# nmwsharp/diffusion-net

Hardware: NVIDIA H100
Metric: DiffusionNetBlock forward Mverts/sec at V=200k,K=128,C=128; 1/2/4/8 GPU (higher is better)
Workload: dtype f32

## Files before the change

### diffusion-net_b200/csrc/dn_tc.cu

```cuda
#include "dn_internal.h"
#include "dn_tc_ptx.cuh"
#include <cuda.h>
#include <cudaTypedefs.h>
#include <cuda_bf16.h>
#include <string.h>

namespace {

using namespace tc;

constexpr int KC = 16;
constexpr int TILE_M = 128;
constexpr int W_RING_BYTES = 128 * 1024;
constexpr int W_NST_MAX = 8;
constexpr int CHAIN_THREADS = 384;
constexpr int A_BOX_BYTES = 8 * TILE_M * 4;
constexpr int A_STAGE_BYTES = 2 * A_BOX_BYTES;
constexpr int A_NST_MAX = 8;
constexpr int SMEM_OPTIN = 232448;
constexpr int OUT_ROWS = 64;
constexpr int OUT_BOX_BYTES = 8 * OUT_ROWS * 4;

enum { MODE_TF32 = 1, MODE_TF32X3 = 3, MODE_BF16 = DN_PASSES_BF16 };

// ... 420 lines not shown
            if (Lr.residual) {
              if (ok0) {
                const float2 r = __ldg(reinterpret_cast<const float2*>(Lr.residual + r0 * Lr.ld_res + col));
                v0.x = fmaf(Lr.res_scale, r.x, v0.x); v0.y = fmaf(Lr.res_scale, r.y, v0.y);
              }
              if (ok1) {
                const float2 r = __ldg(reinterpret_cast<const float2*>(Lr.residual + r1 * Lr.ld_res + col));
                v1.x = fmaf(Lr.res_scale, r.x, v1.x); v1.y = fmaf(Lr.res_scale, r.y, v1.y);
              }
            }
            if (Lr.out) {
              if (ok0) *reinterpret_cast<float2*>(Lr.out + r0 * Lr.ld_out + col) = v0;
              if (ok1) *reinterpret_cast<float2*>(Lr.out + r1 * Lr.ld_out + col) = v1;
            }
          }
          if constexpr (kChain) {
            if (!keep_act) {
              act[8 * j + 4 * h] = v0.x; act[8 * j + 4 * h + 1] = v0.y;
              act[8 * j + 4 * h + 2] = v1.x; act[8 * j + 4 * h + 3] = v1.y;
            }
          }
          if (!kChain && head) {
#pragma unroll
            for (int o = 0; o < (kChain ? 1 : 8); ++o) {
              if (o >= p.head_n) break;
              const float2 w = __ldg(reinterpret_cast<const float2*>(p.head_w + (int64_t)o * N + col));
              hp0[o] = fmaf(w.y, v0.y, fmaf(w.x, v0.x, hp0[o]));
              hp1[o] = fmaf(w.y, v1.y, fmaf(w.x, v1.x, hp1[o]));
            }
          }
        }
      }
      if constexpr (kStage) {
        if (Lr.out || Lr.residual) {
          fence_proxy_async();
          named_bar_sync(2 + wg, 128);
          if (Lr.out && elected && row0 < p.V) {
            for (int b = 0; b < Lr.N / 8; ++b)
              tma_tile_2d_s2g(&p.omap[l], 8 * b, row0, smem_u32(stg_box(b)));
            bulk_commit();
            if (tile + gridDim.x >= ntiles) bulk_wait<0>();
          }
        }
      }
      if (head) {
        auto head_store = [&](int o, float a0, float a1) {
          a0 += __shfl_xor_sync(0xffffffffu, a0, 1);
          a0 += __shfl_xor_sync(0xffffffffu, a0, 2);
          a1 += __shfl_xor_sync(0xffffffffu, a1, 1);
          a1 += __shfl_xor_sync(0xffffffffu, a1, 2);
          const float b = p.head_b ? __ldg(p.head_b + o) : 0.f;
          if (t == 0 && ok0) p.head_out[r0 * p.ld_head_out + o] = a0 + b;
          if (t == 0 && ok1) p.head_out[r1 * p.ld_head_out + o] = a1 + b;
        };
        if constexpr (kChain) {
#pragma unroll 1
          for (int o = 0; o < p.head_n; ++o) {
            float a0 = 0.f, a1 = 0.f;
#pragma unroll
            for (int j = 0; j < NB; ++j) {
              if (j >= nb) break;
#pragma unroll
              for (int h = 0; h < 2; ++h) {
                const float* v = act + 8 * j + 4 * h;
                const float2 w = __ldg(reinterpret_cast<const float2*>(p.head_w + (int64_t)o * N + 16 * j + 8 * h + 2 * t));
                a0 = fmaf(w.y, v[1], fmaf(w.x, v[0], a0));
                a1 = fmaf(w.y, v[3], fmaf(w.x, v[2], a1));
              }
            }
            head_store(o, a0, a1);
          }
        } else {
#pragma unroll
          for (int o = 0; o < (kChain ? 1 : 8); ++o) {
            if (o >= p.head_n) break;
            head_store(o, hp0[o], hp1[o]);
          }
        }
      }
    }
  }
}

constexpr int TB_NST = 4;
constexpr int TB_RAW_HALF = KC * 128 * 4;
constexpr int TB_RAW = 2 * TB_RAW_HALF;
constexpr int TB_BIMG = KC * 128 * 4;
constexpr int TB_BSTAGE = 2 * TB_BIMG;
constexpr int TB_THREADS = 288;
constexpr int TB_SUMS = 64 * 256 * 4;
constexpr int TB_SMEM = TB_NST * TB_RAW + 2 * TB_BSTAGE + TB_SUMS + 256;
constexpr int TB_FOLD = 8;

struct TcToBasisParams {
  const float* values;
  const float* basis;
  const float* mass;
  float* partial;
  int64_t V;
  int K, C;
  int64_t chunks_per_cta;
  int64_t ld_values;
  int64_t ldp;
  const int32_t* cta_rows;
};

template <int MODE, int NBC>
__global__ void __launch_bounds__(TB_THREADS, 1) to_basis_kernel(const __grid_constant__ TcToBasisParams p) {
  extern __shared__ __align__(1024) uint8_t smem[];
  uint8_t* raw = smem;
  uint8_t* bimg = smem + TB_NST * TB_RAW;
  float* sums = reinterpret_cast<float*>(bimg + 2 * TB_BSTAGE);
  uint64_t* bars = reinterpret_cast<uint64_t*>(bimg + 2 * TB_BSTAGE + TB_SUMS);
  const uint32_t st_full = smem_u32(bars), st_empty = smem_u32(bars + TB_NST);
  const int warp = threadIdx.x >> 5, lane = threadIdx.x & 31;
  if (threadIdx.x == 0) {
    for (int i = 0; i < TB_NST; ++i) { mbar_init(st_full + 8 * i, 1); mbar_init(st_empty + 8 * i, 8); }
    fence_barrier_init();
  }
  __syncthreads();

  int64_t rb, re;
  if (p.cta_rows) {
    rb = p.cta_rows[2 * blockIdx.x];
    re = p.cta_rows[2 * blockIdx.x + 1];
  } else {
    rb = (int64_t)blockIdx.x * p.chunks_per_cta * KC;
    re = rb + p.chunks_per_cta * KC;
    if (re > p.V) re = p.V;
  }
  const int64_t nch = re > rb ? (re - rb + KC - 1) / KC : 0;
  constexpr int C = 16 * NBC;
  const int K = p.K;

  if (warp == 8) {
    if (lane == 0) {
      for (int64_t c = 0; c < nch; ++c) {
        const uint32_t s = c % TB_NST, ph = (c / TB_NST) & 1;
        mbar_wait(st_empty + 8 * s, ph ^ 1);
        const int64_t v0 = rb + c * KC;
        const int nv = (int)((re - v0) < KC ? (re - v0) : KC);
        const uint32_t ba = (uint32_t)nv * K * 4, bb = (uint32_t)nv * C * 4;
        mbar_arrive_expect_tx(st_full + 8 * s, ba + bb);
        tma_bulk_g2s(smem_u32(raw + s * TB_RAW), p.basis + v0 * K, ba, st_full + 8 * s);
        if (p.ld_values == C) {
          tma_bulk_g2s(smem_u32(raw + s * TB_RAW + TB_RAW_HALF), p.values + v0 * C, bb, st_full + 8 * s);
        } else {
          for (int j = 0; j < nv; ++j)
            tma_bulk_g2s(smem_u32(raw + s * TB_RAW + TB_RAW_HALF) + (uint32_t)j * C * 4, p.values + (v0 + j) * p.ld_values,
                         (uint32_t)C * 4, st_full + 8 * s);
        }
      }
    }
    return;
  }

  const int g = lane >> 2, t = lane & 3;
  const int m0 = (warp >> 2) * 64 + (warp & 3) * 16 + g;
  const uint32_t lbo = (uint32_t)C * 16;
  float acc[64];
  float* sum = sums + threadIdx.x;
#pragma unroll
  for (int i = 0; i < 64; ++i) sum[256 * i] = 0.f;

  for (int64_t c = 0; c < nch; ++c) {
    const uint32_t s = c % TB_NST, ph = (c / TB_NST) & 1;
    const int64_t v0 = rb + c * KC;
    const int nv = (int)((re - v0) < KC ? (re - v0) : KC);
    const int fold = (int)(c % TB_FOLD);
    if (fold == 0 && c > 0) {
      wgmma_wait<0>();
#pragma unroll
      for (int j = 0; j < 8; ++j) fence_acc8(acc + 8 * j);
#pragma unroll
      for (int i = 0; i < 64; ++i) sum[256 * i] += acc[i];
    }
    float mv[NBC], xv[NBC];
    if (p.mass) {
#pragma unroll
      for (int i = 0; i < NBC; ++i) {
        const int vv = (256 * i + (int)threadIdx.x) / C;
        mv[i] = __ldg(p.mass + v0 + (vv < nv ? vv : nv - 1));
      }
    }
    named_bar_sync(1, 256);
    mbar_wait(st_full + 8 * s, ph);
    const float* rphi = reinterpret_cast<const float*>(raw + s * TB_RAW);
    const float* rx = reinterpret_cast<const float*>(raw + s * TB_RAW + TB_RAW_HALF);
    uint8_t* bh = bimg + (c & 1) * TB_BSTAGE;
#pragma unroll
    for (int i = 0; i < NBC; ++i) xv[i] = rx[256 * i + (int)threadIdx.x];
#pragma unroll
    for (int i = 0; i < NBC; ++i) {
      const int e = 256 * i + (int)threadIdx.x;
      const int vv = e / C, cc = e - vv * C;
      float x = 0.f;
      if (vv < nv) x = p.mass ? xv[i] * mv[i] : xv[i];
      float hi, lo;
      split_tf32_fast(x, hi, lo);
      const uint32_t off = (vv >> 2) * C * 16 + (cc >> 3) * 128 + (cc & 7) * 16 + (vv & 3) * 4;
      *reinterpret_cast<float*>(bh + off) = hi;
      if (MODE == MODE_TF32X3) *reinterpret_cast<float*>(bh + TB_BIMG + off) = lo;
    }
    wgmma_wait<0>();
    uint32_t ah[2][4], al[2][4];
#pragma unroll
    for (int ks = 0; ks < 2; ++ks)
#pragma unroll
      for (int i = 0; i < 4; ++i) {
        const int vv = 8 * ks + t + 4 * (i >> 1), k = m0 + 8 * (i & 1);
        const float v = rphi[vv * K + k];
        float h, lo;
        split_tf32_fast((vv < nv && k < K) ? v : 0.f, h, lo);
        ah[ks][i] = __float_as_uint(h);
        al[ks][i] = __float_as_uint(lo);
      }
    fence_proxy_async();
    __syncwarp();
    if (lane == 0) mbar_arrive(st_empty + 8 * s);
    named_bar_sync(2, 256);
    const uint32_t sb = smem_u32(bh);
#pragma unroll
    for (int ks = 0; ks < 2; ++ks) {
      fence_frag4(ah[ks]);
      if (MODE == MODE_TF32X3) fence_frag4(al[ks]);
    }
    wgmma_fence();
#pragma unroll
    for (int ks = 0; ks < 2; ++ks) {
      const uint32_t acc0 = (fold > 0 || ks > 0) ? 1u : 0u;
      if constexpr (NBC == 8) {
        const uint32_t base = sb + ks * 2 * lbo;
        const uint64_t dh = make_desc(base, lbo, 128);
        if (MODE == MODE_TF32X3) {
          wgmma_tf32_n128(acc, al[ks], dh, acc0);
          wgmma_tf32_n128(acc, ah[ks], make_desc(base + TB_BIMG, lbo, 128), 1u);
          wgmma_tf32_n128(acc, ah[ks], dh, 1u);
        } else {
          wgmma_tf32_n128(acc, ah[ks], dh, acc0);
        }
      } else {
#pragma unroll
        for (int j = 0; j < NBC; ++j) {
          const uint32_t base = sb + ks * 2 * lbo + j * 256;
          const uint64_t dh = make_desc(base, lbo, 128);
          if (MODE == MODE_TF32X3) {
            wgmma_tf32_n16(acc + 8 * j, al[ks], dh, acc0);
            wgmma_tf32_n16(acc + 8 * j, ah[ks], make_desc(base + TB_BIMG, lbo, 128), 1u);
            wgmma_tf32_n16(acc + 8 * j, ah[ks], dh, 1u);
          } else {
            wgmma_tf32_n16(acc + 8 * j, ah[ks], dh, acc0);
          }
        }
      }
    }
    wgmma_commit();
  }
  wgmma_wait<0>();
#pragma unroll
  for (int j = 0; j < 8; ++j) fence_acc8(acc + 8 * j);
  if (nch > 0)
#pragma unroll
    for (int i = 0; i < 64; ++i) sum[256 * i] += acc[i];
  float* out = p.partial + (int64_t)blockIdx.x * K * p.ldp;
#pragma unroll
  for (int b = 0; b < 16; ++b) {
    const int col = 8 * b + 2 * t;
    if (col >= C) break;
    if (m0 < K) *reinterpret_cast<float2*>(out + (int64_t)m0 * p.ldp + col) = make_float2(sum[256 * (4 * b)], sum[256 * (4 * b + 1)]);
    if (m0 + 8 < K)
      *reinterpret_cast<float2*>(out + (int64_t)(m0 + 8) * p.ldp + col) = make_float2(sum[256 * (4 * b + 2)], sum[256 * (4 * b + 3)]);
  }
}

constexpr int kMaxDev = 64;
struct DevState { int queried, sms, sm90, tc_tried, tc; };
DevState g_dev[kMaxDev];

template <typename F>
bool set_smem(F* f, int bytes) {
  return cudaFuncSetAttribute(f, cudaFuncAttributeMaxDynamicSharedMemorySize, bytes) == cudaSuccess;
}
template <int MODE, int NBC0 = 1>
bool set_to_basis_smem() {
  if constexpr (NBC0 > 8) return true;
  else return set_smem(to_basis_kernel<MODE, NBC0>, TB_SMEM) && set_to_basis_smem<MODE, NBC0 + 1>();
}
template <int MODE, int NBC0 = 1>
void launch_to_basis(int nbc, int grid, const TcToBasisParams& p, cudaStream_t st) {
  if constexpr (NBC0 <= 8) {
    if (nbc == NBC0) to_basis_kernel<MODE, NBC0><<<grid, TB_THREADS, TB_SMEM, st>>>(p);
    else launch_to_basis<MODE, NBC0 + 1>(nbc, grid, p, st);
  }
}
template <int MODE>
bool set_chain_smem() {
  constexpr int s128 = ChainRing<MODE, 128>::SMEM, s256 = ChainRing<MODE, 256>::SMEM;
  return set_smem(rows_chain_kernel<MODE, 128, false>, s128) && set_smem(rows_chain_kernel<MODE, 128, true>, s128) &&
         set_smem(rows_chain_kernel<MODE, 256, false>, s256) && set_smem(rows_chain_kernel<MODE, 256, true>, s256);
}

PFN_cuTensorMapEncodeTiled_v12000 tensor_map_encoder() {
  static const PFN_cuTensorMapEncodeTiled_v12000 fn = [] {
    void* f = nullptr;
    cudaDriverEntryPointQueryResult q;
    if (cudaGetDriverEntryPointByVersion("cuTensorMapEncodeTiled", &f, 12000, cudaEnableDefault, &q) != cudaSuccess ||
        q != cudaDriverEntryPointSuccess) {
      cudaGetLastError();
      f = nullptr;
    }
    return reinterpret_cast<PFN_cuTensorMapEncodeTiled_v12000>(f);
  }();
  return fn;
}

}

static DevState* cur_dev_state() {
  int dev = 0;
  if (cudaGetDevice(&dev) != cudaSuccess || dev < 0 || dev >= kMaxDev) {
    cudaGetLastError();
    return nullptr;
  }
  DevState& d = g_dev[dev];
  if (!d.queried) {
    d.queried = 1;
    int major = 0, minor = 0;
    if (cudaDeviceGetAttribute(&d.sms, cudaDevAttrMultiProcessorCount, dev) != cudaSuccess ||
        cudaDeviceGetAttribute(&major, cudaDevAttrComputeCapabilityMajor, dev) != cudaSuccess ||
        cudaDeviceGetAttribute(&minor, cudaDevAttrComputeCapabilityMinor, dev) != cudaSuccess) {
      cudaGetLastError();
      major = 0;
    }
    if (d.sms < 1) d.sms = 1;
    d.sm90 = major == 9 && minor == 0;
  }
  return &d;
}

int dn_sm_count() {
  const DevState* d = cur_dev_state();
  return d ? d->sms : 1;
}

// ... 99 lines not shown
  }
}

int tc_rows_chain(const DnRowsSrc& src, const DnLayer* layers_in, int n_layers, int64_t V, int passes, void* ws,
                  int64_t ws_bytes, cudaStream_t st) {
  if (V <= 0) return DN_OK;
  if (n_layers < 1 || n_layers > DN_MAX_LAYERS) return DN_ERR_INVALID_ARGUMENT;
  DnLayer layers[DN_MAX_LAYERS];
  bool packed = true;
  for (int l = 0; l < n_layers; ++l) {
    layers[l] = layers_in[l];
    packed = packed && layers[l].prepacked != nullptr;
  }
  if (!packed) {
    int rc = tc_pack_layers(layers, n_layers, ws, ws_bytes, nullptr, st);
    if (rc) return rc;
  }
  const bool bf16 = passes == DN_PASSES_BF16 && layers[0].pack_fmt == 2;
  if (passes == DN_PASSES_BF16 && !bf16) passes = 1;
  if (V >= (1ll << 31) - 256) return DN_ERR_UNSUPPORTED;
  HcParams p;
  memset(&p, 0, sizeof(p));
  p.src = src;
  p.n_layers = n_layers;
  p.V = V;
  p.tile_group = layers[0].tile_group;
  p.group_stride = layers[0].group_stride;
  const PFN_cuTensorMapEncodeTiled_v12000 encode = tensor_map_encoder();
  if (!encode) return DN_ERR_UNSUPPORTED;
  auto encode_rows = [&](CUtensorMap* m, const float* base, int width, int64_t ld, int box_rows) {
    const cuuint64_t dims[2] = {(cuuint64_t)width, (cuuint64_t)V};
    const cuuint64_t strides[1] = {(cuuint64_t)ld * 4};
    const cuuint32_t box[2] = {8, (cuuint32_t)box_rows}, estr[2] = {1, 1};
    return encode(m, CU_TENSOR_MAP_DATA_TYPE_FLOAT32, 2, const_cast<float*>(base), dims, strides, box, estr,
                  CU_TENSOR_MAP_INTERLEAVE_NONE, CU_TENSOR_MAP_SWIZZLE_NONE, CU_TENSOR_MAP_L2_PROMOTION_L2_256B,
                  CU_TENSOR_MAP_FLOAT_OOB_FILL_NONE) == CUDA_SUCCESS;
  };
  for (int s = 0; s < src.nsrc; ++s)
    if (!encode_rows(&p.amap[s], src.ptr[s], src.width[s], src.ld[s], TILE_M)) return DN_ERR_UNSUPPORTED;
  int nmax = 0, nmin = 1 << 30;
  for (int l = 0; l < n_layers; ++l) {
    const DnLayer& L = layers[l];
    HcLayer& T = p.layer[l];
    T.wpack = L.prepacked; T.bias = L.bias; T.emul = L.emul; T.relu_mask = L.relu_mask_src; T.row_scale = L.row_scale;
    T.residual = L.residual; T.ld_res = L.ld_res; T.res_scale = L.res_scale; T.out = L.out; T.ld_out = L.ld_out;
    T.K = L.K; T.N = L.N; T.relu = L.relu; T.sibling = L.sibling;
    if (L.N > nmax) nmax = L.N;
    if (L.N < nmin) nmin = L.N;
  }
  if (nmax <= 128 && !bf16)
    for (int l = 0; l < n_layers; ++l) {
      const DnLayer& L = layers[l];
      if (L.out && !encode_rows(&p.omap[l], L.out, L.N, L.ld_out, OUT_ROWS)) return DN_ERR_UNSUPPORTED;
      if (L.residual && !encode_rows(&p.rmap[l], L.residual, L.N, L.ld_res, OUT_ROWS)) return DN_ERR_UNSUPPORTED;
    }
  const bool wide = nmin == nmax && (nmax == 128 || nmax == 256);
  const DnLayer& Ll = layers[n_layers - 1];
  p.head_w = Ll.head_w; p.head_b = Ll.head_b; p.head_out = Ll.head_out; p.ld_head_out = Ll.ld_head_out; p.head_n = Ll.head_n;
  const int64_t ntiles = (V + TILE_M - 1) / TILE_M;
  const int sms = dn_sm_count();
  const int grid = (int)(ntiles < sms ? ntiles : sms);
  if (bf16) launch_chain<MODE_BF16>(p, nmax, wide, grid, st);
  else if (passes == 3) launch_chain<MODE_TF32X3>(p, nmax, wide, grid, st);
  else launch_chain<MODE_TF32>(p, nmax, wide, grid, st);
  DN_LAUNCH_CHECK();
  return DN_OK;
}

int tc_to_basis_supported(int K, int C) {
  if (K % 4 || K < 4 || K > 128) return DN_ERR_UNSUPPORTED;
  if (C % 16 || C < 16 || C > 128) return DN_ERR_UNSUPPORTED;
  return DN_OK;
}

int tc_to_basis_partial(const float* values, const float* basis, const float* massvec, int64_t V, int K, int C,
                        float* partial, int* P_out, int passes, cudaStream_t st, int64_t ld_values, int64_t ldp,
                        const int32_t* cta_rows, int n_ctas) {
  if (tc_to_basis_supported(K, C) != DN_OK) return DN_ERR_UNSUPPORTED;
  if (ld_values <= 0) ld_values = C;
  if (ldp <= 0) ldp = C;
  if ((reinterpret_cast<uintptr_t>(values) & 15) || (reinterpret_cast<uintptr_t>(basis) & 15) || (ld_values % 4) ||
      (ldp % 2) || (reinterpret_cast<uintptr_t>(partial) & 7))
    return DN_ERR_UNSUPPORTED;
  TcToBasisParams p;
  p.values = values; p.basis = basis; p.mass = massvec; p.partial = partial;
  p.ld_values = ld_values; p.ldp = ldp; p.cta_rows = cta_rows;
  p.V = V; p.K = K; p.C = C; p.chunks_per_cta = 0;
  int grid;
  if (cta_rows) {
    if (n_ctas < 1) return DN_ERR_INVALID_ARGUMENT;
    grid = n_ctas;
  } else {
    const int64_t total_chunks = (V + KC - 1) / KC;
    grid = dn_sm_count();
    if (total_chunks < grid) grid = (int)(total_chunks > 0 ? total_chunks : 1);
    p.chunks_per_cta = (total_chunks + grid - 1) / grid;
    if (p.chunks_per_cta < 1) p.chunks_per_cta = 1;
    grid = (int)((total_chunks + p.chunks_per_cta - 1) / p.chunks_per_cta);
    if (grid < 1) grid = 1;
  }
  if (passes == 3) launch_to_basis<MODE_TF32X3>(C / 16, grid, p, st);
  else launch_to_basis<MODE_TF32>(C / 16, grid, p, st);
  DN_LAUNCH_CHECK();
  *P_out = grid;
  return DN_OK;
}
```

### diffusion-net_b200/layers.py

```python
from __future__ import annotations

import torch
import torch.nn as nn

from . import ops


class LearnedTimeDiffusion(nn.Module):

    def __init__(self, C_inout, method='spectral'):
        super(LearnedTimeDiffusion, self).__init__()
        self.C_inout = C_inout
        self.diffusion_time = nn.Parameter(torch.Tensor(C_inout))
        self.method = method
        nn.init.constant_(self.diffusion_time, 0.0)

    def forward(self, x, L, mass, evals, evecs):
        if x.shape[-1] != self.C_inout:
            raise ValueError(
                "Tensor has wrong shape = {}. Last dim shape should have number of channels = {}".format(
                    x.shape, self.C_inout))
        if self.method == 'spectral':
            ops._require_cuda(x, mass, evals, evecs, self.diffusion_time)
            if x.dim() == 2:
# ... 30 lines not shown
        return self.A.weight, None

    def forward(self, vectors):
        ops._require_cuda(vectors)
        A_re, A_im = self.weights()
        lead = vectors.shape[:-3]
        v = vectors.reshape((-1,) + tuple(vectors.shape[-3:]))
        needs_grad = torch.is_grad_enabled() and (vectors.requires_grad or A_re.requires_grad or
                                                  (A_im is not None and A_im.requires_grad))
        outs = []
        for b in range(v.shape[0]):
            if not needs_grad:
                outs.append(ops.spatial_gradient_features_raw(v[b], A_re, A_im))
            else:
                g0, g1 = v[b][..., 0].contiguous(), v[b][..., 1].contiguous()
                lin = lambda w, g: ops.mlp_apply([g], [w], [None])
                if A_im is not None:
                    b_re = lin(A_re, g0) - lin(A_im, g1)
                    b_im = lin(A_re, g1) + lin(A_im, g0)
                else:
                    b_re, b_im = lin(A_re, g0), lin(A_re, g1)
                outs.append(torch.tanh(g0 * b_re + g1 * b_im))
        return torch.stack(outs, 0).reshape(lead + outs[0].shape)


FUSE_HEAD = True


class MiniMLP(nn.Sequential):

    def __init__(self, layer_sizes, dropout=False, activation=nn.ReLU, name="miniMLP"):
        super(MiniMLP, self).__init__()
        self._fused_ok = activation is nn.ReLU
        self._uses_dropout = bool(dropout)
        self._linear_names = []
        for i in range(len(layer_sizes) - 1):
            is_last = (i + 2 == len(layer_sizes))
            if dropout and i > 0:
                self.add_module(name + "_mlp_layer_dropout_{:03d}".format(i), nn.Dropout(p=.5))
            self.add_module(name + "_mlp_layer_{:03d}".format(i), nn.Linear(layer_sizes[i], layer_sizes[i + 1]))
            self._linear_names.append(name + "_mlp_layer_{:03d}".format(i))
            if not is_last:
                self.add_module(name + "_mlp_act_{:03d}".format(i), activation())

    def linears(self):
        return [getattr(self, n) for n in self._linear_names]

    def forward_sources(self, srcs, residual=None):
        lins = self.linears()
        if not self._fused_ok:
            x = torch.cat(srcs, dim=-1)
            for m in self:
                x = ops.mlp_apply([x], [m.weight], [m.bias]) if isinstance(m, nn.Linear) else m(x)
            return x if residual is None else x + residual
        drop_p = 0.5 if (self._uses_dropout and self.training) else 0.0
        return ops.mlp_apply(srcs, [l.weight for l in lins], [l.bias for l in lins], residual=residual,
                             drop_p=drop_p)

    def forward(self, x):
        ops._require_cuda(x)
        lead = x.shape[:-1]
        y = self.forward_sources([x.reshape(-1, x.shape[-1])])
        return y.reshape(lead + (y.shape[-1],))


class DiffusionNetBlock(nn.Module):

    def __init__(self, C_width, mlp_hidden_dims, dropout=True, diffusion_method='spectral',
                 with_gradient_features=True, with_gradient_rotations=True):
        super(DiffusionNetBlock, self).__init__()
        self.C_width = C_width
        self.mlp_hidden_dims = mlp_hidden_dims
        self.dropout = dropout
        self.with_gradient_features = with_gradient_features
        self.with_gradient_rotations = with_gradient_rotations
        self.diffusion = LearnedTimeDiffusion(self.C_width, method=diffusion_method)
        self.MLP_C = 2 * self.C_width
        if self.with_gradient_features:
            self.gradient_features = SpatialGradientFeatures(
                self.C_width, with_gradient_rotations=self.with_gradient_rotations)
            self.MLP_C += self.C_width
        self.mlp = MiniMLP([self.MLP_C] + self.mlp_hidden_dims + [self.C_width], dropout=self.dropout)

    def _forward_mesh(self, x_in, mass, evals, evecs, gops, fused, head=None, lap=None):
        A_re = A_im = None
        if self.with_gradient_features:
            A_re, A_im = self.gradient_features.weights()
        if fused:
            lins = self.mlp.linears()
            return ops.block_forward_raw(x_in, mass, evals, evecs, gops, self.diffusion.diffusion_time, A_re, A_im,
                                         [l.weight for l in lins], [l.bias for l in lins],
                                         self.with_gradient_features, head=head)
        if head is not None:
            raise ops.HeadNotFused()
        x_diffuse = self.diffusion(x_in, lap, mass, evals, evecs)
        srcs = [x_in, x_diffuse]
        if self.with_gradient_features:
            srcs.append(ops.GradFeaturesFn.apply(x_diffuse, A_re, A_im, gops))
        return self.mlp.forward_sources(srcs, residual=x_in)

    def _forward_batch(self, batch, x_in):
        x_diffuse = ops.BatchedDiffusionFn.apply(x_in, self.diffusion.diffusion_time, batch)
        srcs = [x_in, x_diffuse]
        if self.with_gradient_features:
            A_re, A_im = self.gradient_features.weights()
            srcs.append(ops.GradFeaturesFn.apply(x_diffuse, A_re, A_im, batch.gops))
        return self.mlp.forward_sources(srcs, residual=x_in)

    def forward(self, x_in, mass, L, evals, evecs, gradX, gradY, head=None):
        B = x_in.shape[0]
        if x_in.shape[-1] != self.C_width:
            raise ValueError(
                "Tensor has wrong shape = {}. Last dim shape should have number of channels = {}".format(
                    x_in.shape, self.C_width))
        ops._require_cuda(x_in, mass, evals, evecs)
        implicit = self.diffusion.method == 'implicit_dense'
        if self.diffusion.method not in ('spectral', 'implicit_dense'):
            self.diffusion(x_in, L, mass, evals, evecs)
        laps = ops.prepare_laplacians(L, B) if implicit else [None] * B
        pick = lambda t, b: None if t is None else t[b]
        gops = [None] * B
        if self.with_gradient_features:
            if isinstance(gradX, (list, tuple)):
                gys = gradY if gradY is not None else [None] * len(gradX)
                gops = [gx if isinstance(gx, ops.GradOperators) else ops.prepare_operators(gx, gy)
                        for gx, gy in zip(gradX, gys)]
            else:
                gops = ops.prepare_operators_batched(gradX, gradY)
        params_need_grad = any(p.requires_grad for p in self.parameters())
        needs_grad = torch.is_grad_enabled() and (x_in.requires_grad or params_need_grad)
        fused = (not implicit) and (not needs_grad) and self.mlp._fused_ok and not (self.training and self.dropout)
        if head is not None and not fused:
            raise ops.HeadNotFused()
        outs = [self._forward_mesh(x_in[b], mass[b], pick(evals, b), pick(evecs, b), gops[b], fused, head, laps[b])
                for b in range(B)]
        return torch.stack(outs, dim=0)


class DiffusionNet(nn.Module):

    def __init__(self, C_in, C_out, C_width=128, N_block=4, last_activation=None, outputs_at='vertices',
                 mlp_hidden_dims=None, dropout=True, with_gradient_features=True, with_gradient_rotations=True,
                 diffusion_method='spectral'):
        super(DiffusionNet, self).__init__()
        self.C_in = C_in
        self.C_out = C_out
        self.C_width = C_width
        self.N_block = N_block
        self.last_activation = last_activation
        self.outputs_at = outputs_at
        if outputs_at not in ['vertices', 'edges', 'faces', 'global_mean']:
            raise ValueError("invalid setting for outputs_at")
        if mlp_hidden_dims == None:
            mlp_hidden_dims = [C_width, C_width]
        self.mlp_hidden_dims = mlp_hidden_dims
        self.dropout = dropout
        self.diffusion_method = diffusion_method
        if diffusion_method not in ['spectral', 'implicit_dense']:
            raise ValueError("invalid setting for diffusion_method")
        self.with_gradient_features = with_gradient_features
        self.with_gradient_rotations = with_gradient_rotations

        self.first_lin = nn.Linear(C_in, C_width)
        self.last_lin = nn.Linear(C_width, C_out)
        self.blocks = []
        for i_block in range(self.N_block):
            block = DiffusionNetBlock(C_width=C_width, mlp_hidden_dims=mlp_hidden_dims, dropout=dropout,
                                      diffusion_method=diffusion_method,
                                      with_gradient_features=with_gradient_features,
                                      with_gradient_rotations=with_gradient_rotations)
            self.blocks.append(block)
            self.add_module("block_" + str(i_block), self.blocks[-1])

    def _linear(self, lin, x):
        B = x.shape[0]
        return torch.stack([ops.mlp_apply([x[b]], [lin.weight], [lin.bias]) for b in range(B)], 0)

    def forward_batch(self, batch, xs):
        if self.diffusion_method != 'spectral':
            raise NotImplementedError("forward_batch: spectral diffusion only")
        elems = None
        if self.outputs_at in ('edges', 'faces'):
            elems = batch.faces if self.outputs_at == 'faces' else batch.edges
            if elems is None:
                raise ValueError("forward_batch with outputs_at='{0}' needs '{0}' in every MeshBatch item".format(
                    self.outputs_at))
        x = self._forward_batch_layout(batch, xs)
        if elems is not None:
            y = x[elems.view(-1)].view(elems.shape + (x.shape[-1],)).mean(dim=1)
            outs = list(torch.split(y, batch.elem_counts(self.outputs_at)))
        else:
            outs = batch.unpack(x)
        if self.outputs_at == 'global_mean':
            res = []
            for b, o in enumerate(outs):
                m = batch.mass[batch.row_begin[b]:batch.row_begin[b] + batch.n_rows[b]]
                res.append((o * (m / m.sum()).unsqueeze(-1)).sum(dim=-2))
            outs = res
        if self.last_activation != None:
            outs = [self.last_activation(o) for o in outs]
        return outs

    def _forward_batch_layout(self, batch, xs):
        x = xs if torch.is_tensor(xs) else batch.pack(xs)
        if x.shape[-1] != self.C_in:
            raise ValueError("DiffusionNet was constructed with C_in={}, but x_in has last dim={}".format(
                self.C_in, x.shape[-1]))
        needs_grad = torch.is_grad_enabled() and (x.requires_grad or any(p.requires_grad for p in self.parameters()))
        dropout = any(blk.training and blk.dropout for blk in self.blocks)
        if needs_grad or dropout:
            x = ops.mlp_apply([x], [self.first_lin.weight], [self.first_lin.bias])
            for blk in self.blocks:
                x = blk._forward_batch(batch, x)
            return ops.mlp_apply([x], [self.last_lin.weight], [self.last_lin.bias])
        return self._forward_batch_fused(batch, x)

# ... 73 lines not shown
```

### diffusion-net_b200/ops.py

```python
from __future__ import annotations

import ctypes as C
import os
import weakref

import torch

from . import _lib

_ENGINES = {"simt": _lib.ENGINE_SIMT, "tc3x": _lib.ENGINE_TC3X, "tc1x": _lib.ENGINE_TC1X, "bf16": _lib.ENGINE_BF16}
_engine = _ENGINES[os.environ.get("DN_B200_ENGINE", "tc3x")]


def set_engine(name: str):
    global _engine
    _engine = _ENGINES[name]


def get_engine() -> str:
    return {v: k for k, v in _ENGINES.items()}[_engine]


def _require_cuda(*tensors):
    for t in tensors:
# ... 385 lines not shown
        return from_basis_raw(_f32c(g), basis, row_scale=massvec), None, None


class FromBasisFn(torch.autograd.Function):

    @staticmethod
    def forward(ctx, values, basis):
        ctx.save_for_backward(basis)
        return from_basis_raw(values, basis)

    @staticmethod
    def backward(ctx, g):
        (basis,) = ctx.saved_tensors
        return to_basis_raw(_f32c(g), basis, None), None


def to_basis(values, basis, massvec):
    if torch.is_grad_enabled():
        _no_operator_grads(("basis", basis), ("massvec", massvec))
        if values.requires_grad:
            return ToBasisFn.apply(values, basis, massvec)
    return to_basis_raw(values, basis, massvec)


def from_basis(values, basis):
    if torch.is_grad_enabled():
        _no_operator_grads(("basis", basis))
        if values.requires_grad:
            return FromBasisFn.apply(values, basis)
    return from_basis_raw(values, basis)


def compute_hks_raw(evals, evecs, scales):
    _require_cuda(evals, evecs, scales)
    evals, evecs, scales = _f32c(evals), _f32c(evecs), _f32c(scales)
    V, K = evecs.shape
    if evals.shape != (K,) or scales.dim() != 1:
        raise ValueError("compute_hks expects evals (K), evecs (V,K), scales (S)")
    S = scales.shape[0]
    out = torch.empty(V, S, dtype=torch.float32, device=evecs.device)
    with torch.cuda.device(evecs.device):
        _lib.check(_lib.load().dn_compute_hks(evals.data_ptr(), evecs.data_ptr(), scales.data_ptr(), V, K, S,
                                              out.data_ptr(), _stream()), "dn_compute_hks")
    return out


def grad_spmm_raw(ops: GradOperators, x):
    x = _f32c(x)
    V, Cc = x.shape
    out = torch.empty(V, Cc, 2, dtype=torch.float32, device=x.device)
    with _on(x):
        _lib.check(_lib.load().dn_grad_spmm(C.byref(ops.csr[0]), x.data_ptr(), V, Cc, out.data_ptr(), _stream()),
                   "dn_grad_spmm")
    return out


def spatial_gradient_features_raw(vectors, A_re, A_im):
    vectors = _f32c(vectors)
    V, Cc, _ = vectors.shape
    out = torch.empty(V, Cc, dtype=torch.float32, device=vectors.device)
    a_re = _f32c(A_re)
    a_im = _f32c(A_im) if A_im is not None else None
    with _on(vectors):
        ws = workspace(V, Cc, Cc, vectors.device)
        _lib.check(_lib.load().dn_spatial_gradient_features_fwd(
            vectors.data_ptr(), a_re.data_ptr(), a_im.data_ptr() if a_im is not None else None,
            1 if a_im is not None else 0, V, Cc, out.data_ptr(), ws.data_ptr(), ws.numel(), _engine, _stream()),
            "dn_spatial_gradient_features_fwd")
    return out


class HeadNotFused(RuntimeError):
    """The linear head cannot ride in this block's MiniMLP epilogue (shape / engine outside the fused chain)."""


PROFILE_STAGES = ("to_basis", "spectral_scale", "pack_weights", "from_basis_pq", "grad_features_gather", "mlp")


def head_fusable(n_out):
    return 1 <= int(n_out) <= 8


def block_forward_raw(x_in, mass, evals, evecs, ops, time, A_re, A_im, weights, biases, with_features,
                      profile=None, head=None, batch_desc=None):
    lib = _lib.load()
    x_in, mass, evals, evecs = _f32c(x_in), _f32c(mass), _f32c(evals), _f32c(evecs)
    V, Cc = x_in.shape
    K = evecs.shape[1]
    out = torch.empty_like(x_in)
    dims = [weights[0].shape[1]] + [w.shape[0] for w in weights]
    wc = [_f32c(w) for w in weights]
    bc = [_f32c(b) if b is not None else None for b in biases]
    a_re = _f32c(A_re) if A_re is not None else None
    a_im = _f32c(A_im) if A_im is not None else None
    wp = _lib.ptr_array([w.data_ptr() for w in wc])
    bp = _lib.ptr_array([b.data_ptr() if b is not None else None for b in bc])
    dm = _lib.int_array(dims)
    prm = _lib.dn_block_params(
        time.data_ptr(), a_re.data_ptr() if a_re is not None else None,
        a_im.data_ptr() if a_im is not None else None, 1 if with_features else 0,
        1 if a_im is not None else 0, len(weights), wp, bp, dm)
    csr = C.byref(ops.csr[0]) if ops is not None else None
    with _on(x_in):
        extra = 0 if batch_desc is None else int(batch_desc.n_meshes) * K * Cc * 8
        ws = workspace(V, K, max(Cc, max(dims[1:])), x_in.device, extra=extra)
        if head is not None or batch_desc is not None:
            hd, hout = None, None
            if head is not None:
                hw = _f32c(head[0])
                hb = _f32c(head[1]) if head[1] is not None else None
                hout = torch.empty(V, hw.shape[0], dtype=torch.float32, device=x_in.device)
                hd = _lib.dn_head(hw.data_ptr(), hb.data_ptr() if hb is not None else None, int(hw.shape[0]),
                                  hout.data_ptr(), int(hw.shape[0]))
            rc = lib.dn_block_fwd_ex(x_in.data_ptr(), mass.data_ptr(), evals.data_ptr(), evecs.data_ptr(), csr, C.byref(prm),
                                     C.byref(batch_desc) if batch_desc is not None else None,
                                     C.byref(hd) if hd is not None else None, V, K, Cc,
                                     None if head is not None else out.data_ptr(), ws.data_ptr(), ws.numel(), _engine,
                                     _stream())
            if rc == -2 and head is not None:
                raise HeadNotFused()
            _lib.check(rc, "dn_block_fwd_ex")
            return hout if head is not None else out
        if profile is not None:
            ms = (C.c_float * 6)()
            _lib.check(lib.dn_block_fwd_profile(x_in.data_ptr(), mass.data_ptr(), evals.data_ptr(), evecs.data_ptr(),
                                                csr, C.byref(prm), V, K, Cc, out.data_ptr(), ws.data_ptr(),
                                                ws.numel(), _engine, _stream(), ms), "dn_block_fwd_profile")
            profile[:] = [float(v) for v in ms]
            return out
        _lib.check(lib.dn_block_fwd(x_in.data_ptr(), mass.data_ptr(), evals.data_ptr(), evecs.data_ptr(), csr,
                                    C.byref(prm), V, K, Cc, out.data_ptr(), ws.data_ptr(), ws.numel(), _engine,
                                    _stream()), "dn_block_fwd")
    return out


class DiffusionFn(torch.autograd.Function):

    @staticmethod
    @_device_guard
    def forward(ctx, x, time, mass, evals, evecs):
        lib = _lib.load()
        x, mass, evals, evecs = _f32c(x), _f32c(mass), _f32c(evals), _f32c(evecs)
        V, Cc = x.shape
        K = evecs.shape[1]
        xd = torch.empty_like(x)
        x_spec = torch.empty(K, Cc, dtype=torch.float32, device=x.device)
        ws = workspace(V, K, Cc, x.device)
        _lib.check(lib.dn_learned_time_diffusion_fwd(x.data_ptr(), mass.data_ptr(), evals.data_ptr(),
                                                     evecs.data_ptr(), time.data_ptr(), V, K, Cc, xd.data_ptr(),
                                                     x_spec.data_ptr(), ws.data_ptr(), ws.numel(), _engine,
                                                     _stream()), "dn_learned_time_diffusion_fwd")
        ctx.save_for_backward(mass, evals, evecs, time.detach().clone(), x_spec)
        return xd

    @staticmethod
    @_device_guard
    def backward(ctx, g):
        lib = _lib.load()
        mass, evals, evecs, time, x_spec = ctx.saved_tensors
        g = _f32c(g)
        V, Cc = g.shape
        K = evecs.shape[1]
        gx = torch.empty_like(g)
        gt = torch.zeros_like(time)
        ws = workspace(V, K, Cc, g.device)
        _lib.check(lib.dn_learned_time_diffusion_bwd(g.data_ptr(), mass.data_ptr(), evals.data_ptr(),
                                                     evecs.data_ptr(), time.data_ptr(), x_spec.data_ptr(), V, K, Cc,
                                                     gx.data_ptr(), gt.data_ptr(), ws.data_ptr(), ws.numel(),
                                                     _engine, _stream()), "dn_learned_time_diffusion_bwd")
        return gx, gt, None, None, None


IMPLICIT_RTOL = 1e-8
IMPLICIT_MAX_ITER = 20000
implicit_last_status = None


def _implicit_call(what, fn, V, Cc, device, args, outs):
    status = torch.empty(2 + 2 * Cc, dtype=torch.float64, device=device)
    ws = torch.empty(int(_lib.load().dn_implicit_diffusion_workspace_bytes(V, Cc)), dtype=torch.uint8, device=device)
    _lib.check(fn(*args, float(IMPLICIT_RTOL), int(IMPLICIT_MAX_ITER), *outs, status.data_ptr(), ws.data_ptr(),
                  ws.numel(), _stream()), what)
    global implicit_last_status
    st = implicit_last_status = status.cpu()
    if st[0] > 0:
        raise RuntimeError("diffusion_net_b200 {}: {} of {} columns did not converge in {} iterations (worst relative "
                           "residual {:.3e}, tolerance {:.1e})".format(what, int(st[0]), Cc, IMPLICIT_MAX_ITER,
                                                                      float(st[2 + Cc:].max()), IMPLICIT_RTOL))
    return st


class ImplicitDiffusionFn(torch.autograd.Function):

    @staticmethod
    @_device_guard
    def forward(ctx, x, time, mass, lap):
        lib = _lib.load()
        x, mass = _f32c(x), _f32c(mass)
        if time.dtype != torch.float32 or not time.is_contiguous():
            raise RuntimeError("diffusion_time must be a contiguous float32 tensor")
        V, Cc = x.shape
        if lap.V != V or mass.shape != (V,) or time.shape != (Cc,):
            raise ValueError("implicit diffusion: x {}, mass {}, time {} and L ({}x{}) do not agree".format(
                tuple(x.shape), tuple(mass.shape), tuple(time.shape), lap.V, lap.V))
        y = torch.empty_like(x)
# ... 181 lines not shown
```

Before: 188.9.

## Load to_basis tiles via 2D TMA tensor maps with 32-row stages

The to_basis kernel now uses 2D tiled TMA boxes of 8 columns by 32 rows for the basis and values instead of flat bulk copies. The stage depth drops to 3 while each stage grows to 32 vertices, and the folding interval is adjusted to match. The box layout lets each thread build its B-image with fixed offsets and read A fragments without a K-strided pattern, and one named barrier per chunk is removed. Separately, the Python batched fused path writes each mesh straight into a preallocated output instead of calling torch.stack. This adds tensor-map encoding on the host for every call and a limit of V below 2^31.

```diff
diff --git a/diffusion-net_b200/csrc/dn_tc.cu b/diffusion-net_b200/csrc/dn_tc.cu
--- a/diffusion-net_b200/csrc/dn_tc.cu
+++ b/diffusion-net_b200/csrc/dn_tc.cu
@@ -526,25 +526,27 @@
   }
 }
 
-constexpr int TB_NST = 4;
-constexpr int TB_RAW_HALF = KC * 128 * 4;
+constexpr int TB_ROWS = 32;
+constexpr int TB_NST = 3;
+constexpr int TB_BOX = TB_ROWS * 8 * 4;
+constexpr int TB_RAW_HALF = 16 * TB_BOX;
 constexpr int TB_RAW = 2 * TB_RAW_HALF;
-constexpr int TB_BIMG = KC * 128 * 4;
+constexpr int TB_BIMG = TB_ROWS * 128 * 4;
 constexpr int TB_BSTAGE = 2 * TB_BIMG;
 constexpr int TB_THREADS = 288;
 constexpr int TB_SUMS = 64 * 256 * 4;
 constexpr int TB_SMEM = TB_NST * TB_RAW + 2 * TB_BSTAGE + TB_SUMS + 256;
-constexpr int TB_FOLD = 8;
+constexpr int TB_FOLD = 128 / TB_ROWS;
+static_assert(TB_SMEM <= 227 * 1024, "to_basis shared memory");
 
 struct TcToBasisParams {
-  const float* values;
-  const float* basis;
+  CUtensorMap phi_map;
+  CUtensorMap x_map;
   const float* mass;
   float* partial;
   int64_t V;
   int K, C;
   int64_t chunks_per_cta;
-  int64_t ld_values;
   int64_t ldp;
   const int32_t* cta_rows;
 };
@@ -573,27 +575,24 @@
     re = rb + p.chunks_per_cta * KC;
     if (re > p.V) re = p.V;
   }
-  const int64_t nch = re > rb ? (re - rb + KC - 1) / KC : 0;
-  constexpr int C = 16 * NBC;
+  const int64_t nst = re > rb ? (re - rb + TB_ROWS - 1) / TB_ROWS : 0;
+  constexpr int C = 16 * NBC, XB = C / 8;
   const int K = p.K;
 
   if (warp == 8) {
     if (lane == 0) {
-      for (int64_t c = 0; c < nch; ++c) {
+      const int kbn = (K + 7) / 8;
+      const uint32_t bytes = (uint32_t)(kbn + XB) * TB_BOX;
+      for (int64_t c = 0; c < nst; ++c) {
         const uint32_t s = c % TB_NST, ph = (c / TB_NST) & 1;
         mbar_wait(st_empty + 8 * s, ph ^ 1);
-        const int64_t v0 = rb + c * KC;
-        const int nv = (int)((re - v0) < KC ? (re - v0) : KC);
-        const uint32_t ba = (uint32_t)nv * K * 4, bb = (uint32_t)nv * C * 4;
-        mbar_arrive_expect_tx(st_full + 8 * s, ba + bb);
-        tma_bulk_g2s(smem_u32(raw + s * TB_RAW), p.basis + v0 * K, ba, st_full + 8 * s);
-        if (p.ld_values == C) {
-          tma_bulk_g2s(smem_u32(raw + s * TB_RAW + TB_RAW_HALF), p.values + v0 * C, bb, st_full + 8 * s);
-        } else {
-          for (int j = 0; j < nv; ++j)
-            tma_bulk_g2s(smem_u32(raw + s * TB_RAW + TB_RAW_HALF) + (uint32_t)j * C * 4, p.values + (v0 + j) * p.ld_values,
-                         (uint32_t)C * 4, st_full + 8 * s);
-        }
+        const int v0 = (int)(rb + c * TB_ROWS);
+        const uint32_t dst = smem_u32(raw + s * TB_RAW);
+        mbar_arrive_expect_tx(st_full + 8 * s, bytes);
+        for (int b = 0; b < kbn; ++b) tma_tile_2d_g2s(dst + b * TB_BOX, &p.phi_map, 8 * b, v0, st_full + 8 * s);
+#pragma unroll
+        for (int b = 0; b < XB; ++b)
+          tma_tile_2d_g2s(dst + TB_RAW_HALF + b * TB_BOX, &p.x_map, 8 * b, v0, st_full + 8 * s);
       }
     }
     return;
@@ -601,59 +600,52 @@
 
   const int g = lane >> 2, t = lane & 3;
   const int m0 = (warp >> 2) * 64 + (warp & 3) * 16 + g;
+  const int abox = m0 >> 3;
   const uint32_t lbo = (uint32_t)C * 16;
+  const int bv = 4 * warp + (lane >> 3);
+  const uint32_t boff = (uint32_t)warp * C * 16 + (lane & 7) * 16 + (lane >> 3) * 4;
   float acc[64];
   float* sum = sums + threadIdx.x;
 #pragma unroll
   for (int i = 0; i < 64; ++i) sum[256 * i] = 0.f;
 
-  for (int64_t c = 0; c < nch; ++c) {
+  for (int64_t c = 0; c < nst; ++c) {
     const uint32_t s = c % TB_NST, ph = (c / TB_NST) & 1;
-    const int64_t v0 = rb + c * KC;
-    const int nv = (int)((re - v0) < KC ? (re - v0) : KC);
+    const int64_t v0 = rb + c * TB_ROWS;
+    const int nv = (int)((re - v0) < TB_ROWS ? (re - v0) : TB_ROWS);
     const int fold = (int)(c % TB_FOLD);
-    if (fold == 0 && c > 0) {
-      wgmma_wait<0>();
-#pragma unroll
-      for (int j = 0; j < 8; ++j) fence_acc8(acc + 8 * j);
-#pragma unroll
-      for (int i = 0; i < 64; ++i) sum[256 * i] += acc[i];
-    }
-    float mv[NBC], xv[NBC];
-    if (p.mass) {
-#pragma unroll
-      for (int i = 0; i < NBC; ++i) {
-        const int vv = (256 * i + (int)threadIdx.x) / C;
-        mv[i] = __ldg(p.mass + v0 + (vv < nv ? vv : nv - 1));
-      }
-    }
-    named_bar_sync(1, 256);
+    float mv = 1.f;
+    if (p.mass) mv = __ldg(p.mass + v0 + (bv < nv ? bv : nv - 1));
     mbar_wait(st_full + 8 * s, ph);
     const float* rphi = reinterpret_cast<const float*>(raw + s * TB_RAW);
     const float* rx = reinterpret_cast<const float*>(raw + s * TB_RAW + TB_RAW_HALF);
     uint8_t* bh = bimg + (c & 1) * TB_BSTAGE;
-#pragma unroll
-    for (int i = 0; i < NBC; ++i) xv[i] = rx[256 * i + (int)threadIdx.x];
-#pragma unroll
-    for (int i = 0; i < NBC; ++i) {
-      const int e = 256 * i + (int)threadIdx.x;
-      const int vv = e / C, cc = e - vv * C;
+    float xv[XB];
+#pragma unroll
+    for (int b = 0; b < XB; ++b) xv[b] = rx[b * (TB_BOX / 4) + 32 * warp + lane];
+#pragma unroll
+    for (int b = 0; b < XB; ++b) {
       float x = 0.f;
-      if (vv < nv) x = p.mass ? xv[i] * mv[i] : xv[i];
+      if (bv < nv) x = p.mass ? xv[b] * mv : xv[b];
       float hi, lo;
       split_tf32_fast(x, hi, lo);
-      const uint32_t off = (vv >> 2) * C * 16 + (cc >> 3) * 128 + (cc & 7) * 16 + (vv & 3) * 4;
-      *reinterpret_cast<float*>(bh + off) = hi;
-      if (MODE == MODE_TF32X3) *reinterpret_cast<float*>(bh + TB_BIMG + off) = lo;
+      *reinterpret_cast<float*>(bh + boff + 128 * b) = hi;
+      if (MODE == MODE_TF32X3) *reinterpret_cast<float*>(bh + TB_BIMG + boff + 128 * b) = lo;
     }
     wgmma_wait<0>();
-    uint32_t ah[2][4], al[2][4];
-#pragma unroll
-    for (int ks = 0; ks < 2; ++ks)
+    if (fold == 0 && c > 0) {
+#pragma unroll
+      for (int j = 0; j < 8; ++j) fence_acc8(acc + 8 * j);
+#pragma unroll
+      for (int i = 0; i < 64; ++i) sum[256 * i] += acc[i];
+    }
+    uint32_t ah[4][4], al[4][4];
+#pragma unroll
+    for (int ks = 0; ks < 4; ++ks)
 #pragma unroll
       for (int i = 0; i < 4; ++i) {
         const int vv = 8 * ks + t + 4 * (i >> 1), k = m0 + 8 * (i & 1);
-        const float v = rphi[vv * K + k];
+        const float v = rphi[(abox + (i & 1)) * (TB_BOX / 4) + vv * 8 + g];
         float h, lo;
         split_tf32_fast((vv < nv && k < K) ? v : 0.f, h, lo);
         ah[ks][i] = __float_as_uint(h);
@@ -662,16 +654,16 @@
     fence_proxy_async();
     __syncwarp();
     if (lane == 0) mbar_arrive(st_empty + 8 * s);
-    named_bar_sync(2, 256);
+    named_bar_sync(1, 256);
     const uint32_t sb = smem_u32(bh);
 #pragma unroll
-    for (int ks = 0; ks < 2; ++ks) {
+    for (int ks = 0; ks < 4; ++ks) {
       fence_frag4(ah[ks]);
       if (MODE == MODE_TF32X3) fence_frag4(al[ks]);
     }
     wgmma_fence();
 #pragma unroll
-    for (int ks = 0; ks < 2; ++ks) {
+    for (int ks = 0; ks < 4; ++ks) {
       const uint32_t acc0 = (fold > 0 || ks > 0) ? 1u : 0u;
       if constexpr (NBC == 8) {
         const uint32_t base = sb + ks * 2 * lbo;
@@ -703,7 +695,7 @@
   wgmma_wait<0>();
 #pragma unroll
   for (int j = 0; j < 8; ++j) fence_acc8(acc + 8 * j);
-  if (nch > 0)
+  if (nst > 0)
 #pragma unroll
     for (int i = 0; i < 64; ++i) sum[256 * i] += acc[i];
   float* out = p.partial + (int64_t)blockIdx.x * K * p.ldp;
@@ -969,9 +961,22 @@
   if ((reinterpret_cast<uintptr_t>(values) & 15) || (reinterpret_cast<uintptr_t>(basis) & 15) || (ld_values % 4) ||
       (ldp % 2) || (reinterpret_cast<uintptr_t>(partial) & 7))
     return DN_ERR_UNSUPPORTED;
+  if (V >= (1ll << 31) - 256) return DN_ERR_UNSUPPORTED;
   TcToBasisParams p;
-  p.values = values; p.basis = basis; p.mass = massvec; p.partial = partial;
-  p.ld_values = ld_values; p.ldp = ldp; p.cta_rows = cta_rows;
+  memset(&p, 0, sizeof(p));
+  const PFN_cuTensorMapEncodeTiled_v12000 encode = tensor_map_encoder();
+  if (!encode) return DN_ERR_UNSUPPORTED;
+  auto encode_rows = [&](CUtensorMap* m, const float* base, int width, int64_t ld) {
+    const cuuint64_t dims[2] = {(cuuint64_t)width, (cuuint64_t)(V > 0 ? V : 1)};
+    const cuuint64_t strides[1] = {(cuuint64_t)ld * 4};
+    const cuuint32_t box[2] = {8, (cuuint32_t)TB_ROWS}, estr[2] = {1, 1};
+    return encode(m, CU_TENSOR_MAP_DATA_TYPE_FLOAT32, 2, const_cast<float*>(base), dims, strides, box, estr,
+                  CU_TENSOR_MAP_INTERLEAVE_NONE, CU_TENSOR_MAP_SWIZZLE_NONE, CU_TENSOR_MAP_L2_PROMOTION_L2_256B,
+                  CU_TENSOR_MAP_FLOAT_OOB_FILL_NONE) == CUDA_SUCCESS;
+  };
+  if (!encode_rows(&p.phi_map, basis, K, K) || !encode_rows(&p.x_map, values, C, ld_values)) return DN_ERR_UNSUPPORTED;
+  p.mass = massvec; p.partial = partial;
+  p.ldp = ldp; p.cta_rows = cta_rows;
   p.V = V; p.K = K; p.C = C; p.chunks_per_cta = 0;
   int grid;
   if (cta_rows) {
diff --git a/diffusion-net_b200/layers.py b/diffusion-net_b200/layers.py
--- a/diffusion-net_b200/layers.py
+++ b/diffusion-net_b200/layers.py
@@ -136,7 +136,7 @@
             self.MLP_C += self.C_width
         self.mlp = MiniMLP([self.MLP_C] + self.mlp_hidden_dims + [self.C_width], dropout=self.dropout)
 
-    def _forward_mesh(self, x_in, mass, evals, evecs, gops, fused, head=None, lap=None):
+    def _forward_mesh(self, x_in, mass, evals, evecs, gops, fused, head=None, lap=None, out=None):
         A_re = A_im = None
         if self.with_gradient_features:
             A_re, A_im = self.gradient_features.weights()
@@ -144,7 +144,7 @@
             lins = self.mlp.linears()
             return ops.block_forward_raw(x_in, mass, evals, evecs, gops, self.diffusion.diffusion_time, A_re, A_im,
                                          [l.weight for l in lins], [l.bias for l in lins],
-                                         self.with_gradient_features, head=head)
+                                         self.with_gradient_features, head=head, out=out)
         if head is not None:
             raise ops.HeadNotFused()
         x_diffuse = self.diffusion(x_in, lap, mass, evals, evecs)
@@ -186,6 +186,13 @@
         fused = (not implicit) and (not needs_grad) and self.mlp._fused_ok and not (self.training and self.dropout)
         if head is not None and not fused:
             raise ops.HeadNotFused()
+        if fused:
+            n_res = self.C_width if head is None else int(head[0].shape[0])
+            res = torch.empty(B, x_in.shape[1], n_res, dtype=torch.float32, device=x_in.device)
+            for b in range(B):
+                self._forward_mesh(x_in[b], mass[b], pick(evals, b), pick(evecs, b), gops[b], fused, head, laps[b],
+                                   out=res[b])
+            return res
         outs = [self._forward_mesh(x_in[b], mass[b], pick(evals, b), pick(evecs, b), gops[b], fused, head, laps[b])
                 for b in range(B)]
         return torch.stack(outs, dim=0)
diff --git a/diffusion-net_b200/ops.py b/diffusion-net_b200/ops.py
--- a/diffusion-net_b200/ops.py
+++ b/diffusion-net_b200/ops.py
@@ -491,12 +491,18 @@
 
 
 def block_forward_raw(x_in, mass, evals, evecs, ops, time, A_re, A_im, weights, biases, with_features,
-                      profile=None, head=None, batch_desc=None):
+                      profile=None, head=None, batch_desc=None, out=None):
     lib = _lib.load()
     x_in, mass, evals, evecs = _f32c(x_in), _f32c(mass), _f32c(evals), _f32c(evecs)
     V, Cc = x_in.shape
     K = evecs.shape[1]
-    out = torch.empty_like(x_in)
+    n_res = Cc if head is None else int(head[0].shape[0])
+    if out is None:
+        out = torch.empty(V, n_res, dtype=torch.float32, device=x_in.device)
+    elif (out.dtype != torch.float32 or out.device != x_in.device or tuple(out.shape) != (V, n_res)
+          or not out.is_contiguous()):
+        raise ValueError("block_forward_raw: out must be a contiguous float32 ({}, {}) tensor on {}".format(
+            V, n_res, x_in.device))
     dims = [weights[0].shape[1]] + [w.shape[0] for w in weights]
     wc = [_f32c(w) for w in weights]
     bc = [_f32c(b) if b is not None else None for b in biases]
@@ -518,9 +524,8 @@
             if head is not None:
                 hw = _f32c(head[0])
                 hb = _f32c(head[1]) if head[1] is not None else None
-                hout = torch.empty(V, hw.shape[0], dtype=torch.float32, device=x_in.device)
                 hd = _lib.dn_head(hw.data_ptr(), hb.data_ptr() if hb is not None else None, int(hw.shape[0]),
-                                  hout.data_ptr(), int(hw.shape[0]))
+                                  out.data_ptr(), int(hw.shape[0]))
             rc = lib.dn_block_fwd_ex(x_in.data_ptr(), mass.data_ptr(), evals.data_ptr(), evecs.data_ptr(), csr, C.byref(prm),
                                      C.byref(batch_desc) if batch_desc is not None else None,
                                      C.byref(hd) if hd is not None else None, V, K, Cc,
@@ -529,7 +534,7 @@
             if rc == -2 and head is not None:
                 raise HeadNotFused()
             _lib.check(rc, "dn_block_fwd_ex")
-            return hout if head is not None else out
+            return out
         if profile is not None:
             ms = (C.c_float * 6)()
             _lib.check(lib.dn_block_fwd_profile(x_in.data_ptr(), mass.data_ptr(), evals.data_ptr(), evecs.data_ptr(),
```

New measurement: 213.5 (median of 6 runs). 1.13x the previous value.
